# sbelharbi/tcam-wsol-video

Measured on AMD Instinct MI355X. Metric: frames/sec CAM+bbox, ResNet50-TCAM 224×224, 1/2/4/8 MI355X, higher is better.
Workload: dtype fp32

## Files before the change

tcam_wsol_video_amd/csrc/conv_x6.hip:

```cpp
#include <vector>

#include "common.h"
#include "s3_util.h"

namespace {

typedef __bf16 bf16x8 __attribute__((ext_vector_type(8)));
typedef __amdgpu_buffer_rsrc_t rsrc_t;

constexpr int BK = 32;
constexpr uint32_t OOB = 0x80000000u;
constexpr int SC1 = 16;

struct SrcX {
    int C, H, W, stride, up2, G;
};

struct ConvX {
    const void* sp[2];
    uint32_t sbytes[2];
    SrcX s[2];
    int c0, Ctot;
    const void* wt;
    uint32_t wbytes;
// ... 1135 lines not shown
        __builtin_amdgcn_s_barrier();
        pre_last();
        compute(stage);
        }
        asm volatile("s_waitcnt lgkmcnt(0)" ::: "memory");
        __syncthreads();
    }

    template <bool PRE>
    static __device__ __forceinline__ void epilogue(const ConvX& p, int m0, int n0,
                                                    const Acc& acc, uint4* lds, const Res& rv) {
        if constexpr (!M16) {
            ConvTile<F, BM, BN, WM, WN, 1>::epilogue32(p, m0, n0, acc);
        } else {
            Epi::template run<PRE>(p, m0, n0, acc, lds, rv);
        }
    }
};

__device__ __forceinline__ long sk_start(long b, long I, long G) { return b * I / G; }

__device__ __forceinline__ long sk_block_of(long x, long I, long G) {
    long b = x * G / I;
    while (b + 1 < G && sk_start(b + 1, I, G) <= x) ++b;
    while (b > 0 && sk_start(b, I, G) > x) --b;
    return b;
}

template <class T, bool SK>
__global__ __launch_bounds__(T::NT) __attribute__((amdgpu_waves_per_eu(T::MIN_WAVES)))
void conv_x6_kernel(ConvX p) {
    constexpr int BM = T::BM_, BN = T::BN_;
    __shared__ uint4 lds[T::LDS_UINT4];
    typename T::Acc acc;

    if constexpr (!SK) {
        const int lb = xcd_remap(blockIdx.x, p.nblocks);
        const int ntn = p.nblocks / p.mtiles;
        int mi, ni;
        if (p.gm > 1) {
            const int per = p.gm * ntn, g = lb / per, r = lb - g * per;
            mi = g * p.gm + r % p.gm;
            ni = r / p.gm;
        } else {
            mi = (p.dbg & 256) ? lb / ntn : lb % p.mtiles;
            ni = (p.dbg & 256) ? lb % ntn : lb / p.mtiles;
        }
        const int m0 = mi * BM, n0 = ni * BN;
        typename T::Res rv;
        T::segment(p, m0, n0, 0, p.nk, acc, lds, [&]() { T::res_load(p, m0, n0, rv); });
        if constexpr (!T::PREFETCH) T::res_load(p, m0, n0, rv);
        T::template epilogue<true>(p, m0, n0, acc, lds, rv);
        return;
    } else {

    __shared__ int s_old;
    const long G = p.sk_grid;
    const long I = (long)p.ntiles_total * p.nk;
    const long b = xcd_remap(blockIdx.x, p.sk_grid);
    const long it0 = sk_start(b, I, G), it1 = sk_start(b + 1, I, G);
    const int tid = threadIdx.x;
    for (long it = it0; it < it1;) {
        const int t = (int)(it / p.nk);
        const int kb = (int)(it - (long)t * p.nk);
        const int ke = (int)min<long>((long)p.nk, kb + (it1 - it));
        const int m0 = (t % p.mtiles) * BM;
        const int n0 = (t / p.mtiles) * BN;
        typename T::Res rv;
        T::segment(p, m0, n0, kb, ke, acc, lds, [] {});
        if (kb == 0 && ke == p.nk) {
            T::template epilogue<false>(p, m0, n0, acc, lds, rv);
            __syncthreads();
        } else {
            const int which = (it == it0) ? 0 : 1;
            const long slot_off = (b * 2 + which) * (long)(T::ACC * T::NT) * 4;
            const rsrc_t rp = make_rsrc(p.sk_part, 0x7fffffff);
#pragma unroll
            for (int r = 0; r < T::ACC; ++r)
                __builtin_amdgcn_raw_buffer_store_b32(
                    __float_as_uint(acc_get<T>(acc, r)), rp,
                    (int)(slot_off + (r * T::NT + tid) * 4), 0, SC1);
            asm volatile("s_waitcnt vmcnt(0)" ::: "memory");
            __syncthreads();
            const long tb = (long)t * p.nk;
            const long b_lo = sk_block_of(tb, I, G), b_hi = sk_block_of(tb + p.nk - 1, I, G);
            if (tid == 0)
                s_old = __hip_atomic_fetch_add(p.sk_cnt + t, 1, __ATOMIC_RELAXED,
                                               __HIP_MEMORY_SCOPE_AGENT);
            __syncthreads();
            if (s_old == (int)(b_hi - b_lo)) {
                if (tid == 0) {
                    __builtin_amdgcn_fence(__ATOMIC_ACQUIRE, "agent");
                    asm volatile("s_waitcnt vmcnt(0)" ::: "memory");
                }
                __syncthreads();
                acc_zero<T>(acc);
                for (long bb = b_lo; bb <= b_hi; ++bb) {
                    const int wh = (sk_start(bb, I, G) >= tb) ? 0 : 1;
                    const long so = (bb * 2 + wh) * (long)(T::ACC * T::NT) * 4;
#pragma unroll
                    for (int r = 0; r < T::ACC; ++r) {
                        acc_set<T>(acc, r,
                                   acc_get<T>(acc, r) +
                                       __builtin_bit_cast(
                                           float, __builtin_amdgcn_raw_buffer_load_b32(
                                                      rp, (int)(so + (r * T::NT + tid) * 4), 0,
                                                      SC1)));
                        if (r % 16 == 15) asm volatile("" ::: "memory");
                    }
                }
                if (tid == 0)
                    __hip_atomic_store(p.sk_cnt + t, 0, __ATOMIC_RELAXED, __HIP_MEMORY_SCOPE_AGENT);
                T::template epilogue<false>(p, m0, n0, acc, lds, rv);
            }
            __syncthreads();
        }
        it += ke - kb;
    }
    }
}


constexpr int kMaxGroup = 4;
struct ConvXG {
    ConvX p[kMaxGroup];
    int bstart[kMaxGroup + 1];
    int n;
};

template <class T>
__global__ __launch_bounds__(T::NT) __attribute__((amdgpu_waves_per_eu(T::MIN_WAVES)))
void conv_x6_group_kernel(ConvXG g) {
    constexpr int BM = T::BM_, BN = T::BN_;
    __shared__ uint4 lds[T::LDS_UINT4];
    typename T::Acc acc;
    const int b = blockIdx.x;
    int i = 0;
#pragma unroll
    for (int j = 1; j < kMaxGroup; ++j) i += (j < g.n && b >= g.bstart[j]) ? 1 : 0;
    const ConvX& p = g.p[i];
    const int t = b - g.bstart[i];
    if (t >= p.nblocks) return;
    const int lb = xcd_remap(t, p.nblocks);
    const int m0 = (lb % p.mtiles) * BM;
    const int n0 = (lb / p.mtiles) * BN;
    typename T::Res rv;
    T::segment(p, m0, n0, 0, p.nk, acc, lds, [&]() { T::res_load(p, m0, n0, rv); });
    if constexpr (!T::PREFETCH) T::res_load(p, m0, n0, rv);
    T::template epilogue<true>(p, m0, n0, acc, lds, rv);
}

constexpr int TH_T = 16, TH_H = TH_T + 2, TH_PX = TH_H * TH_H;

template <class F, int MB, int GCM = 4>
__global__ __launch_bounds__(256) void conv3x3_thin_kernel(ConvX p) {
    constexpr int TM = MB == 0 ? 1 : 2 * MB;
    constexpr int NP = F::NP, PL = F::PL;
    using V8 = typename F::V8;
    __shared__ uint4 hs[NP * GCM * TH_PX];
    const int tid = threadIdx.x, lane = tid & 63;
    const int w = __builtin_amdgcn_readfirstlane(tid >> 6);
    const int tx = (p.Wout + TH_T - 1) / TH_T, ty = (p.Hout + TH_T - 1) / TH_T;
    const int bid = blockIdx.x;
    const int b = bid / (tx * ty);
    const int rr = bid - b * tx * ty;
    const int oy0 = (rr / tx) * TH_T, ox0 = (rr % tx) * TH_T;
    const int q = lane >> 4, c16 = lane & 15;
    const int arow = 8 * (c16 >> 2) + (c16 & 3);
    const rsrc_t rw = make_rsrc(p.wt, p.wbytes);
    const rsrc_t rs0 = make_rsrc(p.sp[0], p.sbytes[0]);
    const rsrc_t rs1 = make_rsrc(p.sp[1], p.sbytes[1]);
    floatx4 acc[TM][4];
#pragma unroll
    for (int i = 0; i < TM; ++i)
#pragma unroll
        for (int j = 0; j < 4; ++j) acc[i][j] = floatx4{0.f, 0.f, 0.f, 0.f};
    const int CC = p.Ctot < 32 ? p.Ctot : 32;
    const int GC = CC / 8;
    const int nchunk = p.Ctot / CC;
    constexpr bool PF = false;
    constexpr int HIT = (TH_PX * GCM + 255) / 256;
    uint4 hv[HIT][NP];
    auto issue = [&](int ch) {
        const int c0 = ch * CC;
        const bool s1 = c0 >= p.c0;
        const int sH = s1 ? p.s[1].H : p.s[0].H, sW = s1 ? p.s[1].W : p.s[0].W;
        const int sup = s1 ? p.s[1].up2 : p.s[0].up2, sG = s1 ? p.s[1].G : p.s[0].G;
        const rsrc_t r = s1 ? rs1 : rs0;
#pragma unroll
        for (int u = 0; u < HIT; ++u) {
            const int it = u * 256 + tid;
            const int g = it % GC, hp = it / GC;
            const int hy = hp / TH_H, hx = hp - hy * TH_H;
            const int iy = oy0 - 1 + hy, ix = ox0 - 1 + hx;
            const int cl = (s1 ? c0 - p.c0 : c0) + 8 * g;
            const bool ok = it < TH_PX * GC && (unsigned)iy < (unsigned)p.Hout &&
                            (unsigned)ix < (unsigned)p.Wout;
            const uint32_t off = ok ? (uint32_t)((((b * sH + (iy >> sup)) * sW +
                                                   (ix >> sup)) * sG + (cl >> 3)) * F::GB)
                                    : OOB;
#pragma unroll
            for (int pp = 0; pp < NP; ++pp) hv[u][pp] = bload16(r, ok ? off + 16u * pp : OOB);
        }
    };
    if (PF) issue(0);
    for (int ch = 0; ch < nchunk; ++ch) {
        const int c0 = ch * CC;
        if (!PF) issue(ch);
        __syncthreads();
#pragma unroll
        for (int u = 0; u < HIT; ++u) {
            const int it = u * 256 + tid;
            if (it < TH_PX * GC) {
                const int g = it % GC, hp = it / GC;
#pragma unroll
                for (int pp = 0; pp < NP; ++pp) hs[(pp * GCM + g) * TH_PX + hp] = hv[u][pp];
            }
        }
        __syncthreads();
        if (PF && ch + 1 < nchunk) issue(ch + 1);
        const int nks = p.Ctot % 32 == 0 ? 9 : p.nk;
        for (int ks = 0; ks < nks; ++ks) {
            const int kb = p.Ctot % 32 == 0 ? ks * (p.Ctot / 32) + ch : ks;
            const int k = 32 * kb + 8 * q;
            const int tap = k / p.Ctot, cg = ((k - tap * p.Ctot) - c0) >> 3;
            const int kh = tap / 3, kw = tap - kh * 3;
            const bool kin = tap < 9;
            V8 fa[TM][NP], fb[4][NP];
#pragma unroll
            for (int i = 0; i < TM; ++i)
#pragma unroll
                for (int pp = 0; pp < NP; ++pp)
                    fa[i][pp] = __builtin_bit_cast(
                        V8, bload16(rw, (uint32_t)(((kb * PL + q * NP + pp) * p.Mpad +
                                                        (MB == 0 ? c16 : 32 * (i >> 1) +
                                                         4 * (i & 1) + arow)) *
                                                       16)));
#pragma unroll
            for (int j = 0; j < 4; ++j) {
                const int hp = (4 * w + j + kh) * TH_H + c16 + kw;
#pragma unroll
                for (int pp = 0; pp < NP; ++pp) {
                    const uint4 v = kin ? hs[(pp * GCM + cg) * TH_PX + hp] : make_uint4(0, 0, 0, 0);
                    fb[j][pp] = __builtin_bit_cast(V8, v);
                }
            }
#pragma unroll
            for (int t = 0; t < F::NTERM; ++t)
#pragma unroll
                for (int i = 0; i < TM; ++i)
#pragma unroll
                    for (int j = 0; j < 4; ++j)
                        acc[i][j] = F::mfma16(fa[i][F::ta(t)], fb[j][F::tb(t)], acc[i][j]);
        }
    }
    uint8_t* outb = reinterpret_cast<uint8_t*>(p.out);
    using O = typename F::Out;
    constexpr int ONP = O::NP;
    if constexpr (MB == 0) {
        const int g = q >> 1, h = q & 1;
        if (g >= p.Gout) return;
        const float4 b4 = *reinterpret_cast<const float4*>(p.bias + 4 * q);
        const float bb[4] = {b4.x, b4.y, b4.z, b4.w};
        float sc[4] = {1.f, 1.f, 1.f, 1.f};
        if constexpr (F::SCALED) {
            const float4 s4 = *reinterpret_cast<const float4*>(p.wscale + 4 * q);
            sc[0] = s4.x; sc[1] = s4.y; sc[2] = s4.z; sc[3] = s4.w;
        }
        bool bad = false;
#pragma unroll
        for (int j = 0; j < 4; ++j) {
            const int oy = oy0 + 4 * w + j, ox = ox0 + c16;
            if (oy >= p.Hout || ox >= p.Wout) continue;
            const int n = (b * p.Hout + oy) * p.Wout + ox;
            const floatx4 a = acc[0][j];
            uint32_t pt[4][ONP];
#pragma unroll
            for (int e = 0; e < 4; ++e) {
                const float x = epi_val<F>(a[e], sc[e], bb[e]);
                const float y = p.relu ? relu_nan(x) : x;
                if constexpr (O::SCALED) bad |= f16_overflow(y);
                O::split(y, pt[e]);
            }
            const uint32_t off = (uint32_t)((n * p.out_gs + p.out_go + g) * O::GB + 8 * h);
#pragma unroll
            for (int pp = 0; pp < ONP; ++pp)
                *reinterpret_cast<uint2*>(outb + off + 16 * pp) =
                    make_uint2(pt[0][pp] | (pt[1][pp] << 16), pt[2][pp] | (pt[3][pp] << 16));
        }
        if constexpr (O::SCALED) {
            if (bad && p.oflow) *p.oflow = 1;
        }
        return;
    }
#pragma unroll
    for (int tb = 0; tb < MB; ++tb) {
    const int g = 4 * tb + q;
    if (g >= p.Gout) continue;
    float bb[8], sc[8];
    load_bias_scale<F>(p, g, bb, sc);
#pragma unroll
    for (int j = 0; j < 4; ++j) {
        const int oy = oy0 + 4 * w + j, ox = ox0 + c16;
        if (oy >= p.Hout || ox >= p.Wout) continue;
        const int n = (b * p.Hout + oy) * p.Wout + ox;
        const floatx4 a0 = acc[2 * tb][j], a1 = acc[2 * tb + 1][j];
        float x[8];
#pragma unroll
        for (int e = 0; e < 4; ++e) {
            x[e] = epi_val<F>(a0[e], sc[e], bb[e]);
            x[4 + e] = epi_val<F>(a1[e], sc[4 + e], bb[4 + e]);
        }
        uint4 o[ONP];
        split_group<O>(p, x, o);
        const uint32_t off = (uint32_t)((n * p.out_gs + p.out_go + g) * O::GB);
#pragma unroll
        for (int pp = 0; pp < ONP; ++pp) *reinterpret_cast<uint4*>(outb + off + 16 * pp) = o[pp];
    }
    }
}

constexpr int BK_T = 14, BK_H = 16;

struct BneckConv {
    const void* wt;
    const float* wscale;
    const float* bias;
    uint32_t wbytes;
    int Mpad;
};

struct BneckArgs {
    const void* x;
    void* out;
    int* oflow;
    uint32_t xbytes;
    int B, H, W, Cin;
    int ds;
    int tx, ty;
    BneckConv c1, c2, c3;
    unsigned long long* dbg;
    int xcd;
};

template <class F>
__device__ __forceinline__ void bk_split(const float (&x)[8], bool& bad, uint4 (&o)[F::NP]) {
    uint32_t pt[8][F::NP];
#pragma unroll
    for (int e = 0; e < 8; ++e) {
        const float y = relu_nan(x[e]);
        if constexpr (F::SCALED) bad |= f16_overflow(y);
        F::split(y, pt[e]);
    }
#pragma unroll
    for (int pp = 0; pp < F::NP; ++pp)
        o[pp] = make_uint4(pt[0][pp] | (pt[1][pp] << 16), pt[2][pp] | (pt[3][pp] << 16),
                           pt[4][pp] | (pt[5][pp] << 16), pt[6][pp] | (pt[7][pp] << 16));
}

template <class F>
__device__ __forceinline__ void bk_bias_scale(const BneckConv& c, int g, float (&bb)[8],
                                              float (&sc)[8]) {
    const float4 b0 = *reinterpret_cast<const float4*>(c.bias + 8 * g);
    const float4 b1 = *reinterpret_cast<const float4*>(c.bias + 8 * g + 4);
    bb[0] = b0.x; bb[1] = b0.y; bb[2] = b0.z; bb[3] = b0.w;
    bb[4] = b1.x; bb[5] = b1.y; bb[6] = b1.z; bb[7] = b1.w;
    if constexpr (F::SCALED) {
        const float4 s0 = *reinterpret_cast<const float4*>(c.wscale + 8 * g);
        const float4 s1 = *reinterpret_cast<const float4*>(c.wscale + 8 * g + 4);
        sc[0] = s0.x; sc[1] = s0.y; sc[2] = s0.z; sc[3] = s0.w;
        sc[4] = s1.x; sc[5] = s1.y; sc[6] = s1.z; sc[7] = s1.w;
    } else {
#pragma unroll
        for (int e = 0; e < 8; ++e) sc[e] = 1.f;
    }
}

template <class F>
__device__ __forceinline__ void bk_frag_a(rsrc_t rw, int Mpad, int kb, int r0, int q, int arow,
                                          halfx8 (&fa)[2][F::NP]) {
#pragma unroll
    for (int i = 0; i < 2; ++i)
#pragma unroll
        for (int pp = 0; pp < F::NP; ++pp)
            fa[i][pp] = __builtin_bit_cast(
                halfx8, bload16(rw, (uint32_t)(((kb * F::PL + q * F::NP + pp) * Mpad + r0 +
                                                4 * i + arow) * 16)));
}

template <class F>
__device__ __forceinline__ void bk_mma(const halfx8 (&fa)[2][F::NP], const halfx8 (&fb)[F::NP],
                                       floatx4& a0, floatx4& a1) {
#pragma unroll
    for (int t = 0; t < F::NTERM; ++t) {
        a0 = F::mfma16(fa[0][F::ta(t)], fb[F::tb(t)], a0);
        a1 = F::mfma16(fa[1][F::ta(t)], fb[F::tb(t)], a1);
    }
}

template <class F, int TR, int NWV, int XB>
__global__ __launch_bounds__(64 * NWV) __attribute__((amdgpu_waves_per_eu(8 / NWV)))
void bottleneck_f16x3_kernel(BneckArgs a) {
    constexpr int NP = F::NP, GB = F::GB;
    constexpr int NT = 64 * NWV;
    constexpr int HP = (TR + 2) * BK_H;
    constexpr int N1S = HP / 16;
    constexpr int VALID = TR * BK_T;
    constexpr int N2S = (VALID + 15) / 16;
    constexpr int N2 = 16 * N2S;
    constexpr int WN = NWV / 2;
    constexpr int J1 = (N1S + WN - 1) / WN, J2 = (N2S + WN - 1) / WN;
// ... 140 lines not shown
        auto ld = [&](int ks, halfx8 (&f)[2][NP]) {
            const int ch = ks / 9, tap = ks - 9 * ch;
            bk_frag_a<F>(rw, a.c2.Mpad, tap * 2 + ch, 32 * wm, q, arow, f);
        };
#pragma unroll
        for (int r = 0; r < AR; ++r) ld(r, fr[r]);
        for (int k0 = 0; k0 < 18; k0 += AR) {
#pragma unroll
            for (int r = 0; r < AR; ++r) {
                const int ks = k0 + r;
                const int ch = ks / 9, tap = ks - 9 * ch;
                const int kh = tap / 3, kw = tap - 3 * kh;
                const int sh = kh * BK_H + kw;
#pragma unroll
                for (int jj = 0; jj < J2; ++jj) {
                    if (wn + WN * jj < N2S) {
                        halfx8 fb[NP];
#pragma unroll
                        for (int pp = 0; pp < NP; ++pp)
                            fb[pp] = __builtin_bit_cast(
                                halfx8, y1[((4 * ch + q) * NP + pp) * HP + hp0[jj] + sh]);
                        bk_mma<F>(fr[r], fb, acc[0][jj], acc[1][jj]);
                    }
                }
                if (ks + AR < 18) ld(ks + AR, fr[r]);
            }
        }
        __syncthreads();
        const int g = 4 * wm + q;
        float bb[8], sc[8];
        bk_bias_scale<F>(a.c2, g, bb, sc);
#pragma unroll
        for (int jj = 0; jj < J2; ++jj) {
            const int j = wn + WN * jj;
            if (j >= N2S) continue;
            const int n = 16 * j + c16;
            uint4 o[NP];
#pragma unroll
            for (int pp = 0; pp < NP; ++pp) o[pp] = make_uint4(0, 0, 0, 0);
            if (n < VALID) {
                float x[8];
#pragma unroll
                for (int e = 0; e < 4; ++e) {
                    x[e] = epi_val<F>(acc[0][jj][e], sc[e], bb[e]);
                    x[4 + e] = epi_val<F>(acc[1][jj][e], sc[4 + e], bb[4 + e]);
                }
                bk_split<F>(x, bad, o);
            }
#pragma unroll
            for (int pp = 0; pp < NP; ++pp) y2[(g * NP + pp) * N2 + n] = o[pp];
        }
    }
    __syncthreads();
    stamp(2);

    {
        const rsrc_t rw = make_rsrc(a.c3.wt, a.c3.wbytes);
        floatx4 acc[RB][2][N2S];
#pragma unroll
        for (int t = 0; t < RB; ++t)
#pragma unroll
            for (int i = 0; i < 2; ++i)
#pragma unroll
                for (int j = 0; j < N2S; ++j) acc[t][i][j] = floatx4{0.f, 0.f, 0.f, 0.f};
        int gp[N2S];
#pragma unroll
        for (int j = 0; j < N2S; ++j) {
            const int n = 16 * j + c16;
            const int oy = n / BK_T, ox = n - oy * BK_T;
            const int gy = oy0 + oy, gx = ox0 + ox;
            gp[j] = (n < VALID && gy < a.H && gx < a.W) ? (b * a.H + gy) * a.W + gx : -1;
        }
        constexpr int BJ = N2S > 7 ? 7 : N2S, NBJ = (N2S + BJ - 1) / BJ;
        uint4 rres[BJ][NP];
        auto res_issue = [&](int t, int j0) {
            const int g = 4 * (RB * wave + t) + q;
#pragma unroll
            for (int jj = 0; jj < BJ; ++jj) {
                const int j = j0 + jj;
                if (j < N2S) {
                    const bool ok = !a.ds && gp[j] >= 0;
                    const uint32_t off = ok ? (uint32_t)((gp[j] * G + g) * GB) : OOB;
#pragma unroll
                    for (int pp = 0; pp < NP; ++pp)
                        rres[jj][pp] = bload16(rx, ok ? off + 16u * pp : OOB);
                }
            }
        };
        res_issue(0, 0);
        const int nk = 2 + (a.ds ? a.Cin / 32 : 0);
        for (int kb = 0; kb < nk; ++kb) {
            halfx8 fa[RB][2][NP];
#pragma unroll
            for (int t = 0; t < RB; ++t)
                bk_frag_a<F>(rw, a.c3.Mpad, kb, 32 * (RB * wave + t), q, arow, fa[t]);
#pragma unroll
            for (int j = 0; j < N2S; ++j) {
                halfx8 fb[NP];
                if (kb < 2) {
#pragma unroll
                    for (int pp = 0; pp < NP; ++pp)
                        fb[pp] = __builtin_bit_cast(
                            halfx8, y2[((4 * kb + q) * NP + pp) * N2 + 16 * j + c16]);
                } else {
                    const uint32_t off =
                        gp[j] >= 0 ? (uint32_t)((gp[j] * G + 4 * (kb - 2) + q) * GB) : OOB;
#pragma unroll
                    for (int pp = 0; pp < NP; ++pp)
                        fb[pp] = __builtin_bit_cast(halfx8,
                                                    bload16(rx, gp[j] >= 0 ? off + 16u * pp : OOB));
                }
#pragma unroll
                for (int t = 0; t < RB; ++t) bk_mma<F>(fa[t], fb, acc[t][0][j], acc[t][1][j]);
            }
        }
        uint8_t* outb = reinterpret_cast<uint8_t*>(a.out);
#pragma unroll
        for (int t = 0; t < RB; ++t) {
            const int g = 4 * (RB * wave + t) + q;
            float bb[8], sc[8];
            bk_bias_scale<F>(a.c3, g, bb, sc);
#pragma unroll
            for (int k = 0; k < NBJ; ++k) {
                if (t > 0 || k > 0) res_issue(t, k * BJ);
#pragma unroll
                for (int jj = 0; jj < BJ; ++jj) {
                    const int j = k * BJ + jj;
                    if (j >= N2S || gp[j] < 0) continue;
                    float x[8];
#pragma unroll
                    for (int e = 0; e < 4; ++e) {
                        x[e] = epi_val<F>(acc[t][0][j][e], sc[e], bb[e]);
                        x[4 + e] = epi_val<F>(acc[t][1][j][e], sc[4 + e], bb[4 + e]);
                    }
                    if (!a.ds) add_group<F>(x, rres[jj]);
                    uint4 o[NP];
                    bk_split<F>(x, bad, o);
                    const long ob = ((long)gp[j] * 32 + g) * GB;
#pragma unroll
                    for (int pp = 0; pp < NP; ++pp)
                        *reinterpret_cast<uint4*>(outb + ob + 16 * pp) = o[pp];
                }
            }
        }
    }
    const unsigned long long msk = __ballot(bad);
    if (msk && a.oflow && lane == __builtin_ctzll(msk)) *a.oflow = 1;
    stamp(3);
}

int g_force_sk = -1;
int g_dbg = getenv("TCAM_X6_DEBUG") ? atoi(getenv("TCAM_X6_DEBUG")) : 0;

template <class F>
void launch_thin(const ConvX& p, long blocks, int Cout, hipStream_t st) {
    const dim3 grid((unsigned)blocks), block(256);
    if (Cout <= 16 && p.Ctot == 16 && !(g_dbg & 32))
        timed_launch(conv3x3_thin_kernel<F, 0, 2>, grid, block, st, p);
    else if (Cout <= 16 && !(g_dbg & 32))
        timed_launch(conv3x3_thin_kernel<F, 0>, grid, block, st, p);
    else if (Cout <= 32) timed_launch(conv3x3_thin_kernel<F, 1>, grid, block, st, p);
    else timed_launch(conv3x3_thin_kernel<F, 2>, grid, block, st, p);
}

bool thin_ok(const ConvX& p, const tcam_conv_src* srcs, int nsrc, bool has_res) {
    if (p.KH != 3 || p.KW != 3 || p.pad_h != 1 || p.pad_w != 1 || p.Cout > 64 || has_res)
        return false;
    if (!(p.Ctot == 16 || p.Ctot % 32 == 0)) return false;
    for (int i = 0; i < nsrc; ++i) {
        if (srcs[i].stride != 1) return false;
        const int h = srcs[i].up2 ? 2 * srcs[i].H : srcs[i].H;
        const int w = srcs[i].up2 ? 2 * srcs[i].W : srcs[i].W;
        if (h != p.Hout || w != p.Wout) return false;
        if (nsrc == 2 && srcs[0].C % 32) return false;
    }
    return true;
}


int tile_band(const ConvX& p) {
    static const int g = [] {
        const char* e = getenv("TCAM_CONV_GM");
        return e ? atoi(e) : 0;
    }();
    if (g > 1 && p.mtiles > g && p.mtiles % g == 0) return g;
    return 0;
}

template <class T>
int launch_t(ConvX& p, hipStream_t st) {
    constexpr int BM = T::BM_, BN = T::BN_;
    p.mtiles = (p.Cout + BM - 1) / BM;
    const int ntiles = (p.N + BN - 1) / BN;
    p.ntiles_total = p.mtiles * ntiles;
    p.nblocks = p.ntiles_total;
    auto kern = conv_x6_kernel<T, false>;
    auto kern_sk = conv_x6_kernel<T, true>;
    static int resident = -1;
    if (resident < 0) {
        int per_cu = 0, dev = 0, cus = 0;
        if (hipGetDevice(&dev) != hipSuccess ||
            hipDeviceGetAttribute(&cus, hipDeviceAttributeMultiprocessorCount, dev) !=
                hipSuccess ||
            hipOccupancyMaxActiveBlocksPerMultiprocessor(&per_cu, kern_sk, T::NT, 0) !=
                hipSuccess)
            return TCAM_E_ARG;
        const int by_lds = (160 * 1024) / (int)(T::LDS_UINT4 * sizeof(uint4) + 16);
        resident = min(per_cu, by_lds) * cus;
    }
    p.sk_grid = 0;
    p.gm = tile_band(p);
    const long iters = (long)p.ntiles_total * p.nk;
    const int fsk = g_force_sk > 0 ? g_force_sk : p.sk_req;
    if (p.sk_part && fsk > 0) {
        const long needed = (long)fsk * 2 * T::ACC * T::NT * 4;
        if (needed <= p.sk_part_bytes && (long)p.ntiles_total * 4 <= SK_CNT_BYTES)
            p.sk_grid = (int)(fsk < iters ? fsk : iters);
    } else if (p.sk_part && g_force_sk < 0 && T::AUTO_SK && resident > 0 &&
               iters >= 2L * resident) {
        const int waves = (p.ntiles_total + resident - 1) / resident;
        const double eff = (double)p.ntiles_total / ((double)waves * resident);
        const long needed = (long)resident * 2 * T::ACC * T::NT * 4;
        if (eff < 0.8 && p.nk >= 32 && needed <= p.sk_part_bytes &&
            (long)p.ntiles_total * 4 <= SK_CNT_BYTES)
            p.sk_grid = resident;
    } else if (p.sk_part && g_force_sk < 0 && !T::AUTO_SK && resident > 0 && p.nk >= 64 &&
               getenv("TCAM_X6_SK_G") &&
               (long)p.ntiles_total * 5 <= (long)resident * 3) {
        const long grid = std::min<long>(resident, iters / 8);
        const long needed = grid * 2 * T::ACC * T::NT * 4;
        if (grid >= 2L * p.ntiles_total && needed <= p.sk_part_bytes &&
            (long)p.ntiles_total * 4 <= SK_CNT_BYTES)
            p.sk_grid = (int)grid;
    }
    if (p.sk_grid) {
        timed_launch(kern_sk, dim3(p.sk_grid), dim3(T::NT), st, p);
    } else {
        timed_launch(kern, dim3(p.nblocks), dim3(T::NT), st, p);
    }
    TCAM_CHECK_LAUNCH();
    return TCAM_OK;
}

template <class T>
int launch_group_t(ConvX* ps, int n, hipStream_t st) {
    constexpr int BM = T::BM_, BN = T::BN_;
    ConvXG g{};
    int b = 0;
    for (int i = 0; i < n; ++i) {
        ConvX& p = ps[i];
        p.mtiles = (p.Cout + BM - 1) / BM;
        p.ntiles_total = p.mtiles * ((p.N + BN - 1) / BN);
        p.nblocks = p.ntiles_total;
        p.sk_grid = 0;
        g.p[i] = p;
        g.bstart[i] = b;
        b += (p.nblocks + 7) / 8 * 8;
    }
    g.bstart[n] = b;
    g.n = n;
    timed_launch(conv_x6_group_kernel<T>, dim3(b), dim3(T::NT), st, g);
    TCAM_CHECK_LAUNCH();
    return TCAM_OK;
}

template <class F, int BM, int BN, int WM, int WN, int STAGES = 1>
int launch(ConvX& p, hipStream_t st) {
    return launch_t<ConvTile<F, BM, BN, WM, WN, STAGES>>(p, st);
}

constexpr int kNumTiles = 42;
constexpr int kThinTile = 27;
int g_force_tile = -1;

bool is_g_tile(int id);

template <class F>
int launch_tile(int id, ConvX& p, hipStream_t st) {
    if constexpr (!std::is_same<typename F::Out, F>::value) {
        switch (id) {
            case 3: return launch<F, 128, 64, 2, 2>(p, st);
            case 15: return launch_t<ConvTileG<F, 128, 128, 4, 2, 3, true>>(p, st);
            case 17: return launch_t<ConvTile<F, 64, 64, 2, 2, 1, true>>(p, st);
            case 18: return launch_t<ConvTile<F, 128, 64, 2, 2, 1, true>>(p, st);
            case 20: return launch_t<ConvTile<F, 64, 128, 2, 2, 1, true>>(p, st);
            case 26: return launch_t<ConvTileG<F, 128, 128, 4, 2, 3, true, false, true>>(p, st);
            case 30: return launch_t<ConvTileG<F, 256, 128, 4, 2, 3, true, false, true>>(p, st);
            default: break;
        }
        if (!is_g_tile(id)) return launch_t<ConvTile<F, 128, 64, 2, 2, 1, true>>(p, st);
        return launch_t<ConvTileG<F, 256, 128, 4, 2, 3, true, false, true>>(p, st);
    } else if constexpr (F::NP == 1) {
        switch (id) {
            case 2: return launch_t<ConvTile<F, 32, 256, 1, 4, 1, true>>(p, st);
            case 3: return launch<F, 128, 64, 2, 2>(p, st);
            case 6: return launch<F, 256, 128, 4, 2, 2>(p, st);
            case 15: return launch_t<ConvTileG<F, 128, 128, 4, 2, 3, true>>(p, st);
            case 17: return launch_t<ConvTile<F, 64, 64, 2, 2, 1, true>>(p, st);
            case 18: return launch_t<ConvTile<F, 128, 64, 2, 2, 1, true>>(p, st);
            case 20: return launch_t<ConvTile<F, 64, 128, 2, 2, 1, true>>(p, st);
            case 26: return launch_t<ConvTileG<F, 128, 128, 4, 2, 3, true, false, true>>(p, st);
            case 31: return launch_t<ConvTileG<F, 256, 256, 4, 2, 3, false, false, true>>(p, st);
            case 32: return launch_t<ConvTileG<F, 128, 256, 2, 4, 3, false, false, true>>(p, st);
            case 38: return launch_t<ConvTileG<F, 256, 256, 4, 2, 4, false, false, true>>(p, st);
            case 39: return launch_t<ConvTileG<F, 256, 256, 4, 2, 4, true, false, true>>(p, st);
            case 40: return launch_t<ConvTileG<F, 256, 256, 4, 2, 4, true, false, true, false,
                                               true>>(p, st);
            case 41: return launch_t<ConvTileG<F, 256, 256, 4, 2, 3, true, false, true, false,
                                               true>>(p, st);
// ... 589 lines not shown
```

tcam_wsol_video_amd/ops.py:

```python
from __future__ import annotations

import ctypes as C
from typing import List, Optional, Sequence, Tuple

import torch

from . import _lib
from ._lib import check, tcam_conv_dst, tcam_conv_prob, tcam_conv_src


_TIMER = None


_EVENT_POOL: list = []
_EVENT_NEXT = 0


def set_launch_timer(timer: Optional[list], reserve: int = 0) -> None:
    global _TIMER, _EVENT_NEXT
    _TIMER = timer
    if timer is not None:
        _EVENT_NEXT = 0
        _grow_event_pool(2 * int(reserve))

# ... 804 lines not shown
                                       wout, kh, kw, ph, pw, 1 if relu else 0, dst, len(couts),
                                       _ptr(ws), 0 if ws is None else ws.numel(), stream),
              "tcam_conv2d_x6_multi")
    if timer is not None:
        _timer_disarm(lib)
        timer.append(("conv", 2.0 * cout * kdim * B * hout * wout, e0, e1,
                      f"M{cout} K{kdim} N{B * hout * wout} k{kh}x{kw} src{len(srcs)} x{len(couts)}"))
    return res


class ConvMember:

    __slots__ = ("src", "wt", "wscale", "bias", "cout", "hout", "wout", "ksize", "pad", "relu",
                 "out", "out_coff")

    def __init__(self, src: ConvSrc, wt: torch.Tensor, bias: torch.Tensor, cout: int,
                 hout: int, wout: int, ksize, pad, relu: bool = True,
                 wscale: Optional[torch.Tensor] = None, out: Optional[torch.Tensor] = None,
                 out_coff: int = 0):
        self.src, self.wt, self.wscale, self.bias = src, wt, wscale, bias
        self.cout, self.hout, self.wout = int(cout), int(hout), int(wout)
        self.ksize, self.pad, self.relu = _pair(ksize), _pair(pad), bool(relu)
        self.out, self.out_coff = out, int(out_coff)


GROUP_MAX = 4


def conv2d_group(members: Sequence[ConvMember], tile: int = -1) -> List[torch.Tensor]:
    lib = _lib.load()
    assert 1 <= len(members) <= GROUP_MAX
    B = members[0].src.t.shape[0]
    fmt = weight_fmt(members[0].wt)
    if fmt == "amp":
        raise NotImplementedError("grouped launches run the x6 / f16x3 formats")
    f16 = fmt == "f16x3"
    lay = FMT_LAYOUT[fmt]
    arr = (tcam_conv_prob * len(members))()
    outs, flops, desc = [], 0.0, []
    for i, m in enumerate(members):
        assert weight_fmt(m.wt) == fmt and m.src.t.shape[0] == B and not m.src.up2
        if f16 and m.wscale is None:
            raise ValueError("f16x3 weights need their per-channel scales (wscale)")
        _dev(m.wt, m.bias, m.wscale, m.src.t)
        src, kdim = _x6_srcs([m.src], B, m.ksize[0], m.ksize[1], fmt)
        if m.out is None:
            out = lay_empty(lay, B, m.hout, m.wout, m.cout, m.wt.device)
        else:
            out = m.out
            assert _lay(out) == lay and tuple(out.shape[:3]) == (B, m.hout, m.wout)
        arr[i] = tcam_conv_prob(src[0], _ptr(m.wt), _ptr(m.wscale) if f16 else None,
                                _ptr(m.bias), _ptr(out), m.cout, m.hout, m.wout, m.ksize[0],
                                m.ksize[1], m.pad[0], m.pad[1], 1 if m.relu else 0,
                                s3_dims(out)[3], m.out_coff)
        outs.append(out)
        flops += 2.0 * m.cout * kdim * B * m.hout * m.wout
        desc.append(f"M{m.cout} K{kdim} N{B * m.hout * m.wout} k{m.ksize[0]}x{m.ksize[1]}")
    timer = _TIMER
    if timer is not None:
        e0, e1 = _timer_events()
        _timer_arm(lib, e0, e1)
    dev = members[0].wt.device
    check(lib.tcam_conv2d_group(arr, len(members), B, 1 if f16 else 0, int(tile),
                                _ptr(f16_overflow_flag(dev)) if f16 else None, _stream()),
          "tcam_conv2d_group")
    if timer is not None:
        _timer_disarm(lib)
        timer.append(("conv", flops, e0, e1, "group[" + " | ".join(desc) + "]"))
    return outs


def maxpool3x3s2_s3(x: torch.Tensor) -> torch.Tensor:
    lib = _lib.load()
    _dev(x)
    B, H, W, Cc = s3_dims(x)
    Ho, Wo = (H - 1) // 2 + 1, (W - 1) // 2 + 1
    out = act_empty(x, B, Ho, Wo, Cc)
    lay = _lay(x)
    check(getattr(lib, f"tcam_maxpool3x3s2_{lay}")(_ptr(x), _ptr(out), B, Cc, H, W, Ho, Wo,
                                                   _stream()), f"tcam_maxpool3x3s2_{lay}")
    return out


def pool_out_size(n: int, k: int, stride: int, pad: int, ceil_mode: bool = False) -> int:
    num = n + 2 * pad - k
    o = (-(-num // stride) if ceil_mode else num // stride) + 1
    if ceil_mode and (o - 1) * stride >= n + pad:
        o -= 1
    return o


def pool2d_s3(x: torch.Tensor, k, stride: int, pad: int, mode: str = "max",
              ceil_mode: bool = False, out: Optional[torch.Tensor] = None,
              out_coff: int = 0) -> torch.Tensor:
    lib = _lib.load()
    _dev(x)
    kh, kw = _pair(k)
    B, H, W, Cc = s3_dims(x)
    Ho = pool_out_size(H, kh, stride, pad, ceil_mode)
    Wo = pool_out_size(W, kw, stride, pad, ceil_mode)
    if out is None:
        out = act_empty(x, B, Ho, Wo, Cc)
    lay = _lay(x)
    assert _lay(out) == lay and tuple(out.shape[:3]) == (B, Ho, Wo)
    check(getattr(lib, f"tcam_pool2d_{lay}")(_ptr(x), _ptr(out), B, Cc, H, W, Ho, Wo, kh, kw,
                                             stride, pad, 0 if mode == "max" else 1,
                                             s3_dims(out)[3], out_coff, _stream()),
          f"tcam_pool2d_{lay}")
    return out


def up2_resize_s3(x: torch.Tensor, size: Tuple[int, int]) -> torch.Tensor:
    lib = _lib.load()
    _dev(x)
    B, H, W, Cc = s3_dims(x)
    out = act_empty(x, B, size[0], size[1], Cc)
    lay = _lay(x)
    check(getattr(lib, f"tcam_up2_resize_{lay}")(_ptr(x), _ptr(out), B, Cc, H, W, size[0],
                                                 size[1], _stream()), f"tcam_up2_resize_{lay}")
    return out


def wgap_s3(x: torch.Tensor, fc_w: torch.Tensor, fc_b: torch.Tensor) -> torch.Tensor:
    lib = _lib.load()
    _dev(x, fc_w, fc_b)
    B, H, W, Cc = s3_dims(x)
    classes = fc_w.shape[0]
    ws = torch.empty(int(lib.tcam_wgap_s3_ws_bytes(B, Cc, H * W)), device=x.device,
                     dtype=torch.uint8)
    out = torch.empty((B, classes), device=x.device, dtype=torch.float32)
    lay = _lay(x)
    check(getattr(lib, f"tcam_wgap_{lay}")(_ptr(x), _ptr(fc_w), _ptr(fc_b), _ptr(out), None,
                                           _ptr(ws), B, Cc, H * W, classes, _stream()),
          f"tcam_wgap_{lay}")
    return out


def seghead_cam_s3(x: torch.Tensor, w: torch.Tensor, b: torch.Tensor, want_fcams: bool = True,
                   want_u8: bool = True, argmax: bool = False):
    lib = _lib.load()
    _dev(x, w, b)
    B, H, W, Cin = s3_dims(x)
    fcams = torch.empty((B, 2, H, W), device=x.device) if want_fcams else None
    cam = torch.empty((B, H, W), device=x.device)
    u8 = torch.empty((B, H, W), device=x.device, dtype=torch.uint8) if want_u8 else None
    lay = _lay(x)
    check(getattr(lib, f"tcam_seghead_cam_{lay}")(_ptr(x), _ptr(w), _ptr(b), _ptr(fcams),
                                                  _ptr(cam), _ptr(u8), B, Cin, H, W,
                                                  1 if argmax else 0, _stream()),
          f"tcam_seghead_cam_{lay}")
    return fcams, cam, u8


def resize_cam(fcams: torch.Tensor, size: Tuple[int, int], want_fcams: bool = True,
               want_u8: bool = True, argmax: bool = False):
    lib = _lib.load()
    _dev(fcams)
    B, _, Hi, Wi = fcams.shape
    Ho, Wo = size
    fo = torch.empty((B, 2, Ho, Wo), device=fcams.device) if want_fcams else None
    cam = torch.empty((B, Ho, Wo), device=fcams.device)
    u8 = torch.empty((B, Ho, Wo), device=fcams.device, dtype=torch.uint8) if want_u8 else None
    check(lib.tcam_resize_cam(_ptr(fcams), _ptr(fo), _ptr(cam), _ptr(u8), B, Hi, Wi, Ho, Wo,
                              1 if argmax else 0, _stream()), "tcam_resize_cam")
    return fo, cam, u8
```

Before: 5604.

## Add weight-register ring prefetch to thin 3x3 conv kernel for FP16

Adds an AR-deep register ring of weight fragments to the thin 3x3 conv kernel. Weights for tap ks+AR are prefetched while MFMAs for tap ks run, with scalar-offset buffer loads and sched barriers, which is meant to hide weight-load latency. The ring path is enabled by default for FP16 formats when Ctot is a multiple of 32, and sets waves_per_eu hints. It also adds debug flags that skip loads or the epilogue, plus a Python hook for setting those debug flags. The ring raises register use, and the waves_per_eu hint may limit occupancy.

```diff
diff --git a/tcam_wsol_video_amd/csrc/conv_x6.hip b/tcam_wsol_video_amd/csrc/conv_x6.hip
--- a/tcam_wsol_video_amd/csrc/conv_x6.hip
+++ b/tcam_wsol_video_amd/csrc/conv_x6.hip
@@ -1311,8 +1311,11 @@
 
 constexpr int TH_T = 16, TH_H = TH_T + 2, TH_PX = TH_H * TH_H;
 
-template <class F, int MB, int GCM = 4>
-__global__ __launch_bounds__(256) void conv3x3_thin_kernel(ConvX p) {
+template <class F, int MB, int GCM = 4, int AR = 0>
+__global__ __launch_bounds__(256)
+__attribute__((amdgpu_waves_per_eu(AR == 0 ? 1 : MB == 2 ? 2 : 3)))
+void conv3x3_thin_kernel(ConvX p) {
+    static_assert(AR == 0 || (GCM == 4 && 9 % AR == 0), "ring: nine taps per 32-channel chunk");
     constexpr int TM = MB == 0 ? 1 : 2 * MB;
     constexpr int NP = F::NP, PL = F::PL;
     using V8 = typename F::V8;
@@ -1342,6 +1345,9 @@
     uint4 hv[HIT][NP];
     auto issue = [&](int ch) {
         const int c0 = ch * CC;
+        if constexpr (AR > 0) {
+            if ((p.dbg & 4096) && ch > 0) return;
+        }
         const bool s1 = c0 >= p.c0;
         const int sH = s1 ? p.s[1].H : p.s[0].H, sW = s1 ? p.s[1].W : p.s[0].W;
         const int sup = s1 ? p.s[1].up2 : p.s[0].up2, sG = s1 ? p.s[1].G : p.s[0].G;
@@ -1362,11 +1368,34 @@
             for (int pp = 0; pp < NP; ++pp) hv[u][pp] = bload16(r, ok ? off + 16u * pp : OOB);
         }
     };
+    V8 fr[AR > 0 ? AR : 1][TM][NP];
+    uint32_t wv[NP];
+#pragma unroll
+    for (int pp = 0; pp < NP; ++pp)
+        wv[pp] = (AR > 0 && (p.dbg & 2048))
+                     ? OOB
+                     : (uint32_t)(((q * NP + pp) * p.Mpad + (MB == 0 ? c16 : arow)) * 16);
+    auto ldw = [&](int ch, int tap, int i, V8 (&f)[NP]) {
+        const int kb = ch < nchunk ? tap * nchunk + ch : 0;
+        const int so = __builtin_amdgcn_readfirstlane(kb * PL * p.Mpad * 16);
+#pragma unroll
+        for (int pp = 0; pp < NP; ++pp)
+            f[pp] = __builtin_bit_cast(
+                V8, __builtin_amdgcn_raw_buffer_load_b128(
+                        rw, (int)(wv[pp] + (32 * (i >> 1) + 4 * (i & 1)) * 16), so, 0));
+    };
+    if constexpr (AR > 0) {
+#pragma unroll
+        for (int r = 0; r < AR; ++r)
+#pragma unroll
+            for (int i = 0; i < TM; ++i) ldw(0, r, i, fr[r][i]);
+    }
     if (PF) issue(0);
     for (int ch = 0; ch < nchunk; ++ch) {
         const int c0 = ch * CC;
         if (!PF) issue(ch);
         __syncthreads();
+        if (AR == 0 || !((p.dbg & 4096) && ch > 0)) {
 #pragma unroll
         for (int u = 0; u < HIT; ++u) {
             const int it = u * 256 + tid;
@@ -1376,8 +1405,36 @@
                 for (int pp = 0; pp < NP; ++pp) hs[(pp * GCM + g) * TH_PX + hp] = hv[u][pp];
             }
         }
+        }
         __syncthreads();
         if (PF && ch + 1 < nchunk) issue(ch + 1);
+        if constexpr (AR > 0) {
+#pragma unroll
+            for (int ks = 0; ks < 9; ++ks) {
+                const int kh = ks / 3, kw = ks - kh * 3;
+                V8 fb[4][NP];
+#pragma unroll
+                for (int j = 0; j < 4; ++j) {
+                    const int hp = (4 * w + j + kh) * TH_H + c16 + kw;
+#pragma unroll
+                    for (int pp = 0; pp < NP; ++pp)
+                        fb[j][pp] = __builtin_bit_cast(V8, hs[(pp * GCM + q) * TH_PX + hp]);
+                }
+                auto& fa = fr[ks % AR];
+                const int ks2 = ks + AR;
+#pragma unroll
+                for (int i = 0; i < TM; ++i) {
+#pragma unroll
+                    for (int t = 0; t < F::NTERM; ++t)
+#pragma unroll
+                        for (int j = 0; j < 4; ++j)
+                            acc[i][j] = F::mfma16(fa[i][F::ta(t)], fb[j][F::tb(t)], acc[i][j]);
+                    ldw(ch + ks2 / 9, ks2 % 9, i, fa[i]);
+                    __builtin_amdgcn_sched_barrier(0);
+                }
+            }
+            continue;
+        }
         const int nks = p.Ctot % 32 == 0 ? 9 : p.nk;
         for (int ks = 0; ks < nks; ++ks) {
             const int kb = p.Ctot % 32 == 0 ? ks * (p.Ctot / 32) + ch : ks;
@@ -1416,6 +1473,9 @@
     uint8_t* outb = reinterpret_cast<uint8_t*>(p.out);
     using O = typename F::Out;
     constexpr int ONP = O::NP;
+    if constexpr (AR > 0) {
+        if (p.dbg & 8192) return;
+    }
     if constexpr (MB == 0) {
         const int g = q >> 1, h = q & 1;
         if (g >= p.Gout) return;
@@ -1862,9 +1922,30 @@
 int g_force_sk = -1;
 int g_dbg = getenv("TCAM_X6_DEBUG") ? atoi(getenv("TCAM_X6_DEBUG")) : 0;
 
+template <class F> constexpr bool kThinRing = false;
+template <> constexpr bool kThinRing<FmtF16> = true;
+
+int num_cus();
+
 template <class F>
 void launch_thin(const ConvX& p, long blocks, int Cout, hipStream_t st) {
     const dim3 grid((unsigned)blocks), block(256);
+    if constexpr (kThinRing<F>) {
+        if (!(g_dbg & 1024) && p.Ctot % 32 == 0) {
+            const bool a1 = g_dbg & 32768;
+            if (Cout <= 16 && !(g_dbg & 32)) {
+                if (a1) timed_launch(conv3x3_thin_kernel<F, 0, 4, 1>, grid, block, st, p);
+                else timed_launch(conv3x3_thin_kernel<F, 0, 4, 3>, grid, block, st, p);
+                return;
+            } else if (Cout <= 32) {
+                timed_launch(conv3x3_thin_kernel<F, 1, 4, 1>, grid, block, st, p);
+                return;
+            } else if (blocks <= 2L * num_cus()) {
+                timed_launch(conv3x3_thin_kernel<F, 2, 4, 1>, grid, block, st, p);
+                return;
+            }
+        }
+    }
     if (Cout <= 16 && p.Ctot == 16 && !(g_dbg & 32))
         timed_launch(conv3x3_thin_kernel<F, 0, 2>, grid, block, st, p);
     else if (Cout <= 16 && !(g_dbg & 32))
diff --git a/tcam_wsol_video_amd/ops.py b/tcam_wsol_video_amd/ops.py
--- a/tcam_wsol_video_amd/ops.py
+++ b/tcam_wsol_video_amd/ops.py
@@ -980,6 +980,10 @@
     return fcams, cam, u8
 
 
+def conv_x6_debug(flags: int) -> None:
+    check(_lib.load().tcam_conv_x6_debug(int(flags)), "tcam_conv_x6_debug")
+
+
 def resize_cam(fcams: torch.Tensor, size: Tuple[int, int], want_fcams: bool = True,
                want_u8: bool = True, argmax: bool = False):
     lib = _lib.load()
```

Result: no change. 5647 (median of 6 runs) (+0.8%).
